# anassinator/pddp

Hardware: AMD Instinct MI355X
Metric: pddp_iterations_per_sec (higher is better)
Workload: dtype f32; 1 GPU; BASELINE.json configs[1]: cartpole n=4 m=1, known-dynamics iLQR, horizon=100, batch=4096 trajectories per GPU, bounds +-10 (eig-clamp + BoxQP branch), 10 line-search alphas; batch_per_gpu=4096, horizon=100, alphas=10, launch_form=10 rounds per launch, rounds_per_launch=10, backward_kernel_variant=0

## Files before the change

pddp_amd/csrc/accept.hpp:

```cpp
#pragma once

#include "pddp_common.hpp"

namespace pddp {

template <typename T>
struct AcceptArgs {
  int B, N, n, m, A;
  const T* Zc;
  const T* Uc;
  const T* Jc;
  const T* gains;
  const int32_t* bwd_status;
  double tol, max_reg;
  int n_iterations;
  T* Z;
  T* U;
  T* gains_acc;
  T* J_opt;
  double* mu;
  double* delta;
  int32_t* state;
  int32_t* iter;
  uint8_t* active;
  uint8_t* fresh;
  int32_t* n_live;
};

constexpr double kMuMin = 1e-6;
constexpr double kDelta0 = 2.0;

constexpr int kAcceptThreads = 64;
constexpr int kMaxAlphas = 16;
constexpr int kLiveShards = 256;


template <typename T>
struct AcceptIn {
  int bstat, iter;
  double mu, delta;
  T J_opt;
};
template <typename T>
PDDP_DEV AcceptIn<T> accept_load(const AcceptArgs<T>& a, int b) {
  AcceptIn<T> in;
  in.bstat = a.bwd_status[b];
  in.mu = a.mu[b];
  in.delta = a.delta[b];
  in.J_opt = a.J_opt[b];
  in.iter = a.iter[b];
  return in;
}

template <typename T>
PDDP_DEV int argmin_first(const T* J, int A, T& Jm_out) {
  int amin = 0;
  T Jm = J[0];
#pragma unroll
  for (int i = 1; i < kMaxAlphas; ++i) {
    const bool take = (i < A) && (Jm == Jm) && (J[i] < Jm || J[i] != J[i]);
    amin = take ? i : amin;
    Jm = take ? J[i] : Jm;
  }
  Jm_out = Jm;
  return amin;
}

template <typename T>
PDDP_DEV int accept_decide(const AcceptArgs<T>& a, int b, const AcceptIn<T>& in,
                           int amin, T J_new, bool& fresh_out) {
  int amin_out = -1;
  double mu = in.mu, delta = in.delta;
  int st;
  bool increase = false;
  if (in.bstat != 0) {
    increase = true;
    st = PDDP_STATE_NOT_PD;
  } else {
    const T J_opt = in.J_opt;
    if (J_new < J_opt) {
      amin_out = amin;
      delta = (delta < 1.0 ? delta : 1.0) / kDelta0;
      mu *= delta;
      if (mu <= kMuMin) mu = 0.0;
      const T rel = abs_(J_opt - J_new) / J_opt;
      st = (rel < (T)a.tol) ? PDDP_STATE_CONVERGED : PDDP_STATE_ACCEPTED;
      a.J_opt[b] = J_new;
    } else {
      increase = true;
      st = PDDP_STATE_REJECTED;
    }
  }
  if (increase) {
    delta = (delta > 1.0 ? delta : 1.0) * kDelta0;
    mu = (kMuMin > mu * delta) ? kMuMin : mu * delta;
    if (mu >= a.max_reg) st = PDDP_STATE_MAX_REG;
  }
  a.mu[b] = mu;
  a.delta[b] = delta;
  a.state[b] = st;
  uint8_t act = 0, fr = 0;
  if (st == PDDP_STATE_NOT_PD || st == PDDP_STATE_REJECTED) {
    act = 1;
  } else if (st == PDDP_STATE_ACCEPTED) {
    if (in.iter < a.n_iterations) {
      a.iter[b] = in.iter + 1;
      act = 1;
      fr = 1;
    }
  }
  a.active[b] = act;
  a.fresh[b] = fr;
  if (act && a.n_live != nullptr)
    atomicAdd(a.n_live + (b & (kLiveShards - 1)), 1);
  fresh_out = fr != 0;
  return amin_out;
}

}
```

pddp_amd/csrc/line_search_lds.hpp:

```cpp
#pragma once

#include <type_traits>
#include "models.hpp"
#include "problem_args.hpp"
#include "accept.hpp"
#include "riccati_n4.hpp"

namespace pddp {

template <typename T>
PDDP_DEV void group_copy(T* dst, const T* src, int count, int l16) {
  constexpr int kDeep = 8;
  for (int o0 = l16; o0 < count; o0 += 16 * kDeep) {
    T tmp[kDeep];
#pragma unroll
    for (int r = 0; r < kDeep; ++r) {
      const int o = o0 + 16 * r;
      tmp[r] = src[o < count ? o : 0];
    }
#pragma unroll
    for (int r = 0; r < kDeep; ++r) {
      const int o = o0 + 16 * r;
      if (o < count) dst[o] = tmp[r];
    }
  }
}

PDDP_DEV void store4(float* p, float a, float b, float c, float d) {
  *reinterpret_cast<float4*>(p) = make_float4(a, b, c, d);
}
PDDP_DEV void store4(double* p, double a, double b, double c, double d) {
  *reinterpret_cast<double2*>(p) = make_double2(a, b);
  *reinterpret_cast<double2*>(p + 2) = make_double2(c, d);
}

template <typename T, int n, int m>
PDDP_DEV void control_law(const T* z, const T* zr, const T* gr, const T* us,
                          T alpha, const T* umin, const T* umax, T* un) {
#pragma unroll
  for (int r = 0; r < m; ++r) {
    T s = T(0);
#pragma unroll
    for (int c = 0; c < n; ++c)
      s = n4::fma_(z[c] - zr[c], gr[m + r * n + c], s);
    const T du = n4::fma_(alpha, gr[r], s);
    const T v = us[r] + du;
    un[r] = clamp_nan(v, umin[r], umax[r]);
  }
}

#ifdef PDDP_WG_TIMELINE
__device__ long long g_search_timeline[1024][12];
#define PDDP_TLS(I)                                                           \
  do {                                                                        \
    if ((threadIdx.x & 255) == 0 && blockIdx.x < 1024)                        \
      g_search_timeline[blockIdx.x][(I) + 4 * (threadIdx.x >> 8)] =           \
          wall_clock64();                                                     \
  } while (0)
#define PDDP_TLS_AT(SLOT)                                                     \
  do {                                                                        \
    if (threadIdx.x == 0 && blockIdx.x < 1024)                                \
      g_search_timeline[blockIdx.x][SLOT] = wall_clock64();                   \
  } while (0)
#else
#define PDDP_TLS(I)
#define PDDP_TLS_AT(SLOT)
#endif

template <typename T>
struct PreStaged {
  const T* Zs;
  const T* Us;
  const T* Gs;
  int status;
  T J_opt;
  T* carry_rows = nullptr;
};
template <typename T, int MODEL, bool FUSED, int WPB, int H, unsigned QM,
          bool DENSE, bool PRE = false>
PDDP_DEV void line_search_lds_body(const ProblemT<T> P,
                                   const LineSearchArgs<T> a,
                                   const AcceptArgs<T> c, T* rec, T* Lout,
                                   unsigned char* smem_raw,
                                   const PreStaged<T> pre,
                                   const unsigned tid = threadIdx.x) {
  using D = ModelDims<MODEL>;
  constexpr int n = D::n, m = D::m;
  constexpr int GS = m + m * n;
  static_assert(H == 1 || (H == 2 && FUSED), "");
  static_assert(!DENSE || (FUSED && H == 1), "");
  static_assert(!PRE || (FUSED && H == 2 && !DENSE), "");
  constexpr int GST = PRE ? GS + m : GS;
  constexpr int UST = PRE ? GS + m : m;
  constexpr int kTailRows = DENSE ? 8 : 4;
  __shared__ int sh_dec[WPB][4][2];
  const int lane = tid & (kWave - 1);
  const int wave_all = tid >> 6;
  const int wave = H == 1 ? wave_all : wave_all % WPB;
  const int hid = H == 1 ? 0 : wave_all / WPB;
  const int grp = lane >> 4, ai = lane & 15;
  const int N = a.N;
  const int per = DENSE ? N * GS : (N + 1) * n + N * m + N * GS;
  T* smem = reinterpret_cast<T*>(smem_raw) + (size_t)wave * 4 * per;
  const int b0 = (blockIdx.x * WPB + wave) * 4;
  PDDP_TLS(0);

  for (int g = 0; g < (PRE ? 0 : 4); ++g) {
    const int bg = b0 + g;
    if (bg >= a.B) break;
    if (H == 2 && (g & 1) != hid) continue;
    if (a.active != nullptr && a.active[bg] == 0) continue;
    T* dst = smem + (size_t)g * per;
    const T* zs = a.Z + (size_t)bg * (N + 1) * n;
    const T* us = a.U + (size_t)bg * N * m;
    const T* gs = a.gains + (size_t)bg * N * GS;
    if constexpr (DENSE) {
      for (int o = lane; o < N * GS; o += kWave) dst[o] = gs[o];
    } else {
      for (int o = lane; o < (N + 1) * n; o += kWave) dst[o] = zs[o];
      for (int o = lane; o < N * m; o += kWave) dst[(N + 1) * n + o] = us[o];
      for (int o = lane; o < N * GS; o += kWave)
        dst[(N + 1) * n + N * m + o] = gs[o];
    }
  }
  if constexpr (!PRE) __syncthreads();
  PDDP_TLS(1);

  const int b = b0 + grp;
  const bool exists = b < a.B;
  const int bc = exists ? b : a.B - 1;
  const bool attempted =
      exists && (a.active == nullptr || a.active[bc] != 0);
  const bool run =
      attempted && ai < a.A &&
      (PRE ? pre.status == 0
           : (a.bwd_status == nullptr || a.bwd_status[bc] == 0));
  if constexpr (!FUSED) {
    if (!run) return;
  }
  const bool bounded = a.u_min != nullptr && a.u_max != nullptr;
  T umin[m], umax[m];
#pragma unroll
  for (int r = 0; r < m; ++r) {
    umin[r] = bounded ? a.u_min[r] : -(T)__builtin_inff();
    umax[r] = bounded ? a.u_max[r] : (T)__builtin_inff();
  }
  const T* Zs = PRE ? pre.Zs
                    : DENSE ? a.Z + (size_t)bc * (N + 1) * n
                            : smem + (size_t)grp * per;
  const T* Us = PRE ? pre.Us
                    : DENSE ? a.U + (size_t)bc * N * m : Zs + (N + 1) * n;
  const T* Gs = PRE ? pre.Gs : DENSE ? smem + (size_t)grp * per : Us + N * m;
  const size_t zstep_c = (size_t)a.A * n, ustep_c = (size_t)a.A * m;
  AcceptIn<T> acc_in = {};
  if constexpr (FUSED) {
    if (attempted && ai == 0) {
      acc_in = accept_load(c, b);
      if constexpr (PRE) {
        acc_in.bstat = pre.status;
        acc_in.J_opt = pre.J_opt;
      }
    }
  }
  T Jmine = T(0);
  const bool nocand = FUSED && n <= 4 && Lout == nullptr && rec != nullptr &&
                      a.drop_candidates != 0 && N + 1 <= 16 * H * kTailRows;
  const bool store_uc = !(FUSED && n <= 6 && Lout == nullptr &&
                          rec != nullptr && N + 1 <= 16 * H * kTailRows);
  auto rollout = [&](T alpha, T* Zci, size_t zstep, T* Uci, size_t ustep) {
    T z[n], zn[n], un[m];
#pragma unroll
    for (int j = 0; j < n; ++j) z[j] = Zs[j];
    T J = T(0);
    auto step = [&](const int t) {
      T zr[n], gr[GS], us[m];
      if constexpr (PRE && n == 4) {
        typedef T V4_ __attribute__((ext_vector_type(4)));
        const V4_ v = *reinterpret_cast<const V4_*>(
            __builtin_assume_aligned(Zs + t * 4, 16));
        zr[0] = v[0]; zr[1] = v[1]; zr[2] = v[2]; zr[3] = v[3];
      } else {
#pragma unroll
        for (int j = 0; j < n; ++j) zr[j] = Zs[t * n + j];
      }
      if constexpr (PRE && GST == 6) {
        typedef T V2_ __attribute__((ext_vector_type(2)));
        const V2_* g2 = reinterpret_cast<const V2_*>(
            __builtin_assume_aligned(Gs + t * 6, 8));
        const V2_ a0 = g2[0], a1 = g2[1], a2 = g2[2];
        gr[0] = a0[0]; gr[1] = a0[1]; gr[2] = a1[0]; gr[3] = a1[1];
        gr[4] = a2[0]; us[0] = a2[1];
      } else {
#pragma unroll
        for (int j = 0; j < GS; ++j) gr[j] = Gs[t * GST + j];
#pragma unroll
        for (int j = 0; j < m; ++j) us[j] = Us[t * UST + j];
      }
      const Trig<T, MODEL> tr = trig_of<T, MODEL>(z);
      __builtin_amdgcn_sched_barrier(0);
      if constexpr (PRE) __builtin_amdgcn_s_waitcnt(0xC07F);
      control_law<T, n, m>(z, zr, gr, us, alpha, umin, umax, un);
#pragma unroll
      for (int j = 0; j < n; ++j) Zci[(size_t)t * zstep + j] = z[j];
      if constexpr (!PRE) {
        if (store_uc) {
#pragma unroll
          for (int j = 0; j < m; ++j) Uci[(size_t)t * ustep + j] = un[j];
        }
      }
      J += cost_value<T, MODEL, QM>(P, z, un, tr, false);
      dynamics<T, MODEL, false>(P, z, un, tr, zn, nullptr, nullptr);
#pragma unroll
      for (int j = 0; j < n; ++j) z[j] = zn[j];
    };
    int t = 0;
    if constexpr (n <= 4) {
      for (; t + 3 < N; t += 4) {
        step(t);
        step(t + 1);
        step(t + 2);
        step(t + 3);
      }
    }
#pragma unroll 1
    for (; t < N; ++t) step(t);
#pragma unroll
    for (int j = 0; j < n; ++j) Zci[(size_t)N * zstep + j] = z[j];
    const T lf =
        cost_value<T, MODEL>(P, z, nullptr, trig_of<T, MODEL>(z), true);
    return J + lf;
  };
  if (run && hid == 0) {
    const T alpha = a.alphas[ai];
    const int idx = b * a.A + ai;
    const bool compact0 = FUSED && Lout == nullptr && rec != nullptr &&
                          ai == 0 && n <= 6 && N + 1 <= 16 * H * kTailRows;
    T* Zci = compact0 ? rec + (size_t)b * (N + 1) * n
                      : a.Zc + ((size_t)b * (N + 1) * a.A + ai) * n;
    T* Uci = a.Uc + ((size_t)b * N * a.A + ai) * m;
    const size_t zstep = compact0 ? (size_t)n : (nocand ? 0 : zstep_c);
    const size_t ustep = nocand ? 0 : ustep_c;
    Jmine = rollout(alpha, Zci, zstep, Uci, ustep);
    a.Jc[idx] = Jmine;
  }
  PDDP_TLS(2);

  if constexpr (FUSED) {
    constexpr int kNone = 99;
    const T kInf = (T)__builtin_inff();
    const int nan_first =
        n4::group_min((run && Jmine != Jmine) ? ai : kNone);
    T Jf = (run && Jmine == Jmine) ? Jmine : kInf;
    {
      T y = n4::dpp<0x128>(Jf); Jf = y < Jf ? y : Jf;
      y = n4::dpp<0x12C>(Jf); Jf = y < Jf ? y : Jf;
      y = n4::dpp<(2 | (3 << 2) | (0 << 4) | (1 << 6))>(Jf); Jf = y < Jf ? y : Jf;
      y = n4::dpp<(1 | (0 << 2) | (3 << 4) | (2 << 6))>(Jf); Jf = y < Jf ? y : Jf;
    }
    const int min_first = n4::group_min((run && Jmine == Jf) ? ai : kNone);
    const int amin =
        nan_first != kNone ? nan_first : (min_first != kNone ? min_first : 0);
    const T J_new = nan_first != kNone ? (T)__builtin_nanf("") : Jf;

    int amin_out = -1, fresh_i = 0;
    if (attempted && ai == 0 && hid == 0) {
      bool fr;
      amin_out = accept_decide(c, b, acc_in, amin, J_new, fr);
      fresh_i = fr ? 1 : 0;
    }
    amin_out = __shfl(amin_out, lane & 48);
    fresh_i = __shfl(fresh_i, lane & 48);
    PDDP_TLS_AT(8);
    if constexpr (n <= 4) {
      if (nocand && hid == 0 && __any(amin_out > 0)) {
        if (amin_out > 0 && ai == amin_out)
          rollout(a.alphas[ai], rec + (size_t)b * (N + 1) * n, (size_t)n,
                  a.Uc + ((size_t)b * N * a.A + ai) * m, 0);
      }
    }
    if constexpr (H == 1) {
      if (!__any(amin_out >= 0)) return;
      __builtin_amdgcn_fence(__ATOMIC_ACQ_REL, "workgroup");
    } else {
      if (hid == 0 && ai == 0) {
        sh_dec[wave][grp][0] = amin_out;
        sh_dec[wave][grp][1] = fresh_i;
      }
      __builtin_amdgcn_fence(__ATOMIC_ACQ_REL, "workgroup");
      __syncthreads();
      amin_out = sh_dec[wave][grp][0];
      fresh_i = sh_dec[wave][grp][1];
    }
    PDDP_TLS_AT(9);
    if (amin_out >= 0) {
      constexpr RecLayout lay(n, m);
      constexpr int S = lay.stride;
      const T* srcz = a.Zc + ((size_t)b * (N + 1) * a.A + amin_out) * n;
      const T* srcu = a.Uc + ((size_t)b * N * a.A + amin_out) * m;
      T* Zb = c.Z + (size_t)b * (N + 1) * n;
      T* Ub = c.U + (size_t)b * N * m;
      T* rec_b = rec + (size_t)b * (N + 1) * S;
      T* Ls = PRE ? nullptr : smem + (size_t)grp * per;
      const T* G = c.gains + (size_t)b * N * GS;
      T* Ga = c.gains_acc + (size_t)b * N * GS;
      T zc[n], uc[m];
      const int t_first = ai + 16 * hid;
      constexpr int KR = kTailRows;
      if (n <= 6 && Lout == nullptr && N + 1 <= 16 * H * KR) {
        T zz[KR][n], uu[KR][m];
        const bool from_rec = rec != nullptr && (amin_out == 0 || nocand);
        const T* cz = from_rec ? rec + (size_t)b * (N + 1) * n : srcz;
        const size_t czs = from_rec ? (size_t)n : zstep_c;
#pragma unroll
        for (int k = 0; k < KR; ++k) {
          const int t = t_first + 16 * H * k;
          const int tz = t <= N ? t : N;
#pragma unroll
          for (int j = 0; j < n; ++j) zz[k][j] = cz[(size_t)tz * czs + j];
        }
        const T* Gl = Gs;
        if constexpr (PRE) {
          for (int t = ai + 16 * hid; t < N; t += 16 * H) {
#pragma unroll
            for (int j = 0; j < GS; ++j) Ga[t * GS + j] = Gl[t * GST + j];
          }
        } else {
          constexpr int kDeep = 8;
          int o = ai + 16 * hid;
          for (; o + 16 * H * (kDeep - 1) < N * GS; o += 16 * H * kDeep) {
            T tmp[kDeep];
#pragma unroll
            for (int r = 0; r < kDeep; ++r) tmp[r] = Gl[o + 16 * H * r];
#pragma unroll
            for (int r = 0; r < kDeep; ++r) Ga[o + 16 * H * r] = tmp[r];
          }
          for (; o < N * GS; o += 16 * H) Ga[o] = Gl[o];
        }
        PDDP_TLS_AT(10);
        const T alpha_w = a.alphas[amin_out];
#pragma unroll
        for (int k = 0; k < KR; ++k) {
          const int t = t_first + 16 * H * k;
          const int tu = t < N ? t : 0;
          T zr[n], gr[GS], us[m];
#pragma unroll
          for (int j = 0; j < n; ++j) zr[j] = Zs[tu * n + j];
#pragma unroll
          for (int j = 0; j < GS; ++j) gr[j] = Gs[tu * GST + j];
#pragma unroll
          for (int j = 0; j < m; ++j) us[j] = Us[tu * UST + j];
          control_law<T, n, m>(zz[k], zr, gr, us, alpha_w, umin, umax, uu[k]);
        }
#pragma unroll
        for (int k = 0; k < KR; ++k) {
          const int t = t_first + 16 * H * k;
          if (t <= N) {
#pragma unroll
            for (int j = 0; j < n; ++j) Zb[t * n + j] = zz[k][j];
          }
          if (t < N) {
#pragma unroll
            for (int j = 0; j < m; ++j) Ub[t * m + j] = uu[k][j];
          }
          if constexpr (PRE) {
            if (pre.carry_rows != nullptr && t <= N && N - t <= 16) {
              T* cr = pre.carry_rows + (N - t) * (n + m);
#pragma unroll
              for (int j = 0; j < n; ++j) cr[j] = zz[k][j];
              if (t < N) {
#pragma unroll
                for (int j = 0; j < m; ++j) cr[n + j] = uu[k][j];
              }
            }
          }
        }
      } else {
      {
        const int tz = t_first <= N ? t_first : N;
        const int tu = t_first < N ? t_first : 0;
#pragma unroll
        for (int j = 0; j < n; ++j) zc[j] = srcz[(size_t)tz * zstep_c + j];
#pragma unroll
        for (int j = 0; j < m; ++j) uc[j] = srcu[(size_t)tu * ustep_c + j];
      }
#pragma unroll 1
      for (int t = t_first; t <= N; t += 16 * H) {
        T zn_[n], un_[m];
        {
          const int t2 = t + 16 * H;
          const int tz = t2 <= N ? t2 : N, tu = t2 < N ? t2 : 0;
#pragma unroll
          for (int j = 0; j < n; ++j) zn_[j] = srcz[(size_t)tz * zstep_c + j];
#pragma unroll
          for (int j = 0; j < m; ++j) un_[j] = srcu[(size_t)tu * ustep_c + j];
        }
        const bool terminal = (t == N);
        T un[m];
#pragma unroll
        for (int j = 0; j < m; ++j) un[j] = terminal ? T(0) : uc[j];
#pragma unroll
        for (int j = 0; j < n; ++j) Zb[t * n + j] = zc[j];
        if (!terminal) {
#pragma unroll
          for (int j = 0; j < m; ++j) Ub[t * m + j] = un[j];
        }
        if (fresh_i && Lout != nullptr) {
          T w[S];
          const T l = record_of<T, MODEL>(P, zc, un, terminal, bounded, a.u_min,
                                         a.u_max, w);
          T* dst = rec_b + (size_t)t * S;
#pragma unroll
          for (int j = 0; j < S; j += 4)
            store4(dst + j, w[j], w[j + 1], w[j + 2], w[j + 3]);
          Lout[(size_t)b * (N + 1) + t] = l;
          Ls[t] = l;
        }
#pragma unroll
        for (int j = 0; j < n; ++j) zc[j] = zn_[j];
#pragma unroll
        for (int j = 0; j < m; ++j) uc[j] = un_[j];
      }
      if constexpr (H == 1) {
        group_copy(Ga, G, N * GS, ai);
      } else {
        const int half = (N * GS + 1) / 2;
        const int off = hid * half;
        const int cnt = hid == 0 ? half : N * GS - half;
        group_copy(Ga + off, G + off, cnt, ai);
      }
      }
      if constexpr (H == 1) {
        if (fresh_i && Lout != nullptr) {
          __builtin_amdgcn_fence(__ATOMIC_RELEASE, "wavefront");
          __builtin_amdgcn_wave_barrier();
          if (ai == 0) {
            T Jacc = T(0);
            for (int t = 0; t <= N; ++t) Jacc += Ls[t];
            c.J_opt[b] = Jacc;
            c.fresh[b] = 0;
          }
        }
      }
    }
    if constexpr (H == 2) {
      __syncthreads();
      if (!PRE && amin_out >= 0 && fresh_i && Lout != nullptr && hid == 0 &&
          ai == 0) {
        const T* Ls = smem + (size_t)grp * per;
        T Jacc = T(0);
        for (int t = 0; t <= N; ++t) Jacc += Ls[t];
        c.J_opt[b] = Jacc;
        c.fresh[b] = 0;
      }
    }
  }
  PDDP_TLS(3);
}


template <typename T, int MODEL, bool FUSED, int WPB, int H = 1,
          unsigned QM = kFullMask<MODEL>, bool DENSE = false>
__global__ __launch_bounds__(kWave * WPB * H) __attribute__((
    amdgpu_waves_per_eu((WPB * H >= 8 || DENSE) && sizeof(T) == 4 &&
                                ModelDims<MODEL>::n <= 4
                            ? 4
                            : 1))) void
line_search_lds_kernel(
    ProblemT<T> P, LineSearchArgs<T> a, AcceptArgs<T> c, T* rec, T* Lout) {
  extern __shared__ __attribute__((aligned(16))) unsigned char smem_raw[];
  line_search_lds_body<T, MODEL, FUSED, WPB, H, QM, DENSE>(
      P, a, c, rec, Lout, smem_raw, PreStaged<T>{});
}

}
```

pddp_amd/csrc/riccati_n4_elem.hpp:

```cpp
#pragma once

#include <type_traits>
#include "models.hpp"
#include "riccati_n4_quad.hpp"

namespace pddp {

namespace n4d {
typedef float f32x4 __attribute__((ext_vector_type(4)));
PDDP_DEV int sgn(float x) { return __float_as_int(x); }
PDDP_DEV int splat(int w) {
  int r;
  asm("v_ashrrev_i32 %0, 31, %1" : "=v"(r) : "v"(w));
  return r;
}
PDDP_DEV float bsel(int mask, float a, float b) {
  float r;
  asm("v_bfi_b32 %0, %1, %2, %3" : "=v"(r) : "v"(mask), "v"(a), "v"(b));
  return r;
}

template <typename T>
struct GenArgs {
  const T* Z;
  const T* U;
  T* L;
  T* J_opt;
  uint8_t* fresh;
};
}

namespace n4e {

using n4::bperm;
using n4::dpp;
using n4::fma_;
using n4::group_sum;
using n4::kGain;
using n4::mul_nc;
using n4d::bsel;
using n4d::f32x4;
typedef float f32x2 __attribute__((ext_vector_type(2)));
typedef float f32x3 __attribute__((ext_vector_type(3)));
using n4d::GenArgs;
using n4d::sgn;
using n4d::splat;

constexpr int kWaves = 4;
constexpr int kTrajW = 4;
constexpr int kBlk = 16;
constexpr int kImg = 52;
constexpr int kRowStride = kBlk * kImg + 16;
constexpr int kImgBuf = kTrajW * kRowStride;
constexpr int kTermRow = 24;
constexpr int kTermSh = kTrajW * kTermRow;
constexpr int kPairLdsInl = kImgBuf;
constexpr int kPairLdsOvl = 2 * kImgBuf + kTermSh;

struct LsTableF {
  float v[n4::kLsSteps];
  constexpr LsTableF() : v() {
    for (int n = 0; n < n4::kLsSteps; ++n) v[n] = (float)n4::kLs.v[n];
  }
};
__device__ constexpr LsTableF kLsF{};
template <typename T>
PDDP_DEV const T* ls_table();
template <>
PDDP_DEV const float* ls_table<float>() { return kLsF.v; }
template <>
PDDP_DEV const double* ls_table<double>() { return n4::kLs.v; }
template <typename T>
struct Vec {
  typedef T v4 __attribute__((ext_vector_type(4)));
  typedef T v2 __attribute__((ext_vector_type(2)));
};

struct QpLean1 {
  float x, inv;
  int free_w;
  PDDP_DEV void solve(float x0, float Q, float c, float lo, float hi) {
    const float d_lo = lo - x0, d_hi = x0 - hi;
    const float xs = __builtin_amdgcn_fmed3f(x0, lo, hi);
    const float hQ = 0.5f * Q;
    inv = __builtin_amdgcn_rcpf(Q);
// ... 127 lines not shown
    T kx = qc.x;
    bool Kzero = !qc.free_, fail = qc.fail;
    const bool slow = qc.slow & take;
    if (__any(slow)) {
      unsigned long long todo = __ballot(slow && l == 0);
      while (todo != 0) {
        const int src = __builtin_ctzll(todo);
        todo &= todo - 1;
        const n4::SlowQpOut<T> o = n4q::boxqp1_wave<T, true>(
            __shfl(kprev, src), __shfl(qp_Q, src), __shfl(Qu, src),
            __shfl(lo_b, src), __shfl(hi_b, src), ls_table<T>(), lane);
        const bool mine = (lane >> 4) == (src >> 4);
        kx = mine ? o.x : kx;
        Kzero = mine ? ((o.result_free & 1) == 0) : Kzero;
        fail = mine ? (o.result_free < 2) : fail;
      }
    }
    const T sx = Kzero ? T(0) : qc.inv;
    const int stt = st != PDDP_BWD_OK ? st : (fail ? (int)PDDP_BWD_BOXQP_FAILED : (int)PDDP_BWD_OK);
    T cx, wx;
    n4q::rank_one_coeffs(kx, sx, Quu, Qu, cx, wx);
    kt = take ? kx : kt; sK = take ? sx : sK;
    c = take ? cx : c; wv = take ? wx : wv;
    const bool bad = take & (stt != PDDP_BWD_OK);
    status = bad ? stt : status;
    alive_m &= ~__ballot(bad);
  }
  return ElemGains<T>{kt, sK, c, wv};
}

#ifdef PDDP_ELEM_MARKS
__device__ long long g_elem_marks[8];
#define PDDP_EM_MARK(I) do { if (blockIdx.x == 0 && threadIdx.x == 0) g_elem_marks[I] = clock64(); } while (0)
#define PDDP_EM_ACC(I, T0) do { if (blockIdx.x == 0 && threadIdx.x == 0) g_elem_marks[I] += clock64() - (T0); } while (0)
#define PDDP_EM_NOW() clock64()
#else
#define PDDP_EM_MARK(I)
#define PDDP_EM_ACC(I, T0)
#define PDDP_EM_NOW() 0
#endif

#ifdef PDDP_WG_TIMELINE
__device__ long long g_elem_timeline[1024][12];
#define PDDP_TL(I)                                                            \
  do {                                                                        \
    if ((threadIdx.x & 255) == 0 && blockIdx.x < 1024)                        \
      g_elem_timeline[blockIdx.x][(I) + 4 * (threadIdx.x >> 8)] =             \
          wall_clock64();                                                     \
  } while (0)
#define PDDP_TL_HW(I)                                                         \
  do {                                                                        \
    if (threadIdx.x == 0 && blockIdx.x < 1024) {                              \
      g_elem_timeline[blockIdx.x][8] =                                        \
          __builtin_amdgcn_s_getreg(4 | (0 << 6) | (31 << 11));               \
      g_elem_timeline[blockIdx.x][9] =                                        \
          __builtin_amdgcn_s_getreg(20 | (0 << 6) | (3 << 11));               \
      g_elem_timeline[blockIdx.x][I] = clock64();                             \
    }                                                                         \
  } while (0)
#else
#define PDDP_TL(I)
#define PDDP_TL_HW(I)
#endif

struct RoundOut {
  const float* Zs;
  const float* Gs;
  const float* Us;
  int status;
  float J_opt;
  float* carry_rows;
};
constexpr int round_zu_stride(int N) { return 4 * (N + 1); }
constexpr int kCarryRows = kBlk + 1, kCarryW = 5;
constexpr int kCarryF = kTrajW * kCarryRows * kCarryW;
constexpr int kGainL = kGain + 1;
constexpr int round_gains_floats(int N) { return (kTrajW * N * kGainL + 3) & ~3; }

template <typename T, unsigned QM, bool OVL, bool ROUND>
PDDP_DEV bool elem_sweep_body(const RiccatiArgs<T>& a, const GenArgs<T>& gen,
                              const ProblemT<T>& prob, unsigned char* smem_raw,
                              RoundOut& ro,
                              const unsigned tid = threadIdx.x,
                              const int carry = -1) {
  static_assert(OVL || !ROUND, "");
  constexpr bool F32 = std::is_same<T, float>::value;
  static_assert(F32 || (!OVL && !ROUND), "");
  using V4 = typename Vec<T>::v4;
  using V2 = typename Vec<T>::v2;
  constexpr int MODEL = PDDP_MODEL_CARTPOLE;
  constexpr RecLayout lay(4, 1);
  const int kPairLds = OVL ? kPairLdsOvl + (ROUND ? round_gains_floats(a.N) +
                                                        (carry >= 0 ? kCarryF : 0)
                                                  : 0)
                           : kPairLdsInl;
  const int lane = tid & (kWave - 1);
  const int wave = __builtin_amdgcn_readfirstlane((int)tid >> 6);
  const int pair = OVL ? (wave & (kWaves - 1)) : wave;
  const bool is_gen = OVL && wave >= kWaves;
  T* const img0 = reinterpret_cast<T*>(smem_raw) + pair * kPairLds;
  T* const term_w = OVL ? img0 + 2 * kImgBuf : img0;

  const int row = lane >> 4, l = lane & 15, i = l >> 2, j = l & 3;
  const int N = a.N;
  const int b0 = (blockIdx.x * kWaves + pair) * kTrajW;
  const int b = b0 + row;
  const bool exists = b < a.B;
  const int bc = exists ? b : a.B - 1;
  const T* Zg = gen.Z + (size_t)bc * (size_t)(N + 1) * 4;
  const T* Ug = gen.U + (size_t)bc * (size_t)N;
  const int nblk = (N + kBlk - 1) / kBlk;
  if (b0 >= a.B) return false;
  const bool counted = exists && (a.active == nullptr || a.active[bc] != 0);
  if (!__any(counted)) return false;
  PDDP_EM_MARK(0);
  PDDP_TL(0);
  PDDP_TL_HW(10);
  const T umin = a.u_min[0], umax = a.u_max[0];
  const int rbase = row * kRowStride;

  T zq[4], uq, Jacc = T(0), l_term = T(0);
  [[maybe_unused]] T* const carry_w =
      img0 + kPairLdsOvl + (ROUND ? round_gains_floats(N) : 0) +
      row * kCarryRows * kCarryW;
  if constexpr (ROUND) ro.carry_rows = carry >= 0 ? carry_w : nullptr;
  auto request = [&](int jb) {
    int tau = N - 1 - kBlk * jb - l;
    tau = tau < 0 ? 0 : tau;
    if constexpr (ROUND) {
      if (jb == 0 && carry == 0) {
        const T* cr = carry_w + (N - tau) * kCarryW;
        zq[0] = cr[0]; zq[1] = cr[1]; zq[2] = cr[2]; zq[3] = cr[3];
        uq = cr[4];
        return;
      }
    }
    const V4 v = *reinterpret_cast<const V4*>(Zg + 4 * tau);
    zq[0] = v[0]; zq[1] = v[1]; zq[2] = v[2]; zq[3] = v[3];
    uq = Ug[tau];
    if constexpr (ROUND) {
      if (jb == 0 && carry == 1 && N - tau <= kBlk) {
        T* cr = carry_w + (N - tau) * kCarryW;
        cr[0] = zq[0]; cr[1] = zq[1]; cr[2] = zq[2]; cr[3] = zq[3];
        cr[4] = uq;
      }
    }
  };
  auto terminal = [&]() {
    T zN[4];
    if (ROUND && carry == 0) {
      zN[0] = carry_w[0]; zN[1] = carry_w[1]; zN[2] = carry_w[2];
      zN[3] = carry_w[3];
    } else {
      const V4 zNv = *reinterpret_cast<const V4*>(Zg + 4 * N);
      zN[0] = zNv[0]; zN[1] = zNv[1]; zN[2] = zNv[2]; zN[3] = zNv[3];
      if (ROUND && carry == 1 && l == 0) {
        carry_w[0] = zN[0]; carry_w[1] = zN[1]; carry_w[2] = zN[2];
        carry_w[3] = zN[3];
      }
    }
    T lz[4], lzz[16], lu[1], luu[1];
    l_term = cost_derivs<T, MODEL>(prob, zN, nullptr, trig_of<T, MODEL>(zN),
                                   true, lz, lzz, lu, luu);
    T* scr = term_w + row * kTermRow;
    if (l == 0) {
#pragma unroll
      for (int k = 0; k < 16; k += 4)
        *reinterpret_cast<V4*>(scr + k) =
            V4{lzz[k], lzz[k + 1], lzz[k + 2], lzz[k + 3]};
      *reinterpret_cast<V4*>(scr + 16) = V4{lz[0], lz[1], lz[2], lz[3]};
      scr[20] = l_term;
      if (counted) gen.L[(size_t)bc * (size_t)(N + 1) + N] = l_term;
    }
  };
  auto pass = [&](int jb, T* buf) {
    const T z[4] = {zq[0], zq[1], zq[2], zq[3]};
    const T u = uq;
    if (jb + 1 < nblk) request(jb + 1);
    const int tau = N - 1 - kBlk * jb - l;
    T w[lay.stride];
    const T lc = record_of<T, MODEL, QM>(prob, z, &u, false, true, a.u_min,
                                         a.u_max, w);
    T* dst = buf + rbase + l * kImg;
#pragma unroll
    for (int r = 0; r < 4; ++r)
      *reinterpret_cast<V4*>(dst + 4 * r) =
          V4{w[lay.oFz + ((r + 0) & 3) * 4 + r],
                w[lay.oFz + ((r + 1) & 3) * 4 + r],
                w[lay.oFz + ((r + 2) & 3) * 4 + r],
                w[lay.oFz + ((r + 3) & 3) * 4 + r]};
#pragma unroll
    for (int x = 0; x < 4; x += 2) {
      *reinterpret_cast<V4*>(dst + 16 + 2 * x) =
          V4{w[lay.oFu + x], w[lay.oLuz + x], w[lay.oFu + x + 1],
                w[lay.oLuz + x + 1]};
      *reinterpret_cast<V4*>(dst + 24 + 2 * x) =
          V4{w[lay.oFu + x], w[lay.oLz + x], w[lay.oFu + x + 1],
                w[lay.oLz + x + 1]};
    }
#pragma unroll
    for (int r = 0; r < 4; ++r)
      *reinterpret_cast<V4*>(dst + 32 + 4 * r) =
          V4{w[lay.oLzz + 4 * r], w[lay.oLzz + 4 * r + 1],
                w[lay.oLzz + 4 * r + 2], w[lay.oLzz + 4 * r + 3]};
    *reinterpret_cast<V4*>(dst + 48) =
        V4{w[lay.oLuu], w[lay.oLu], umin - w[lay.oU], umax - w[lay.oU]};
    if (tau >= 0) {
      if (counted) gen.L[(size_t)bc * (size_t)(N + 1) + tau] = lc;
      Jacc += lc;
    }
  };
  auto finish_costs = [&]() {
    const bool sums = counted && (gen.fresh == nullptr || gen.fresh[bc] != 0);
    const T Jrow = group_sum(Jacc) + (OVL ? term_w[row * kTermRow + 20] : l_term);
    if constexpr (ROUND) {
      const T Jold = gen.J_opt[bc];
      if (l == 0) term_w[row * kTermRow + 21] = sums ? Jrow : Jold;
    }
    if (sums && l == 0) {
      gen.J_opt[bc] = Jrow;
      if (gen.fresh != nullptr) gen.fresh[bc] = 0;
    }
  };
  [[maybe_unused]] T* const gains_w = img0 + kPairLdsOvl;
  auto flush_gains = [&](const T* ib, int t_top, int cnt) {
    const T* sg = ib + l * kImg + rbase;
    const V4 Kv = *reinterpret_cast<const V4*>(sg);
    const T kv = sg[4];
    if (exists && l < cnt) {
      T* g = a.gains + ((size_t)bc * (size_t)N + (size_t)(t_top - l)) * kGain;
      g[0] = kv; g[1] = Kv[0]; g[2] = Kv[1]; g[3] = Kv[2]; g[4] = Kv[3];
      if constexpr (ROUND) {
        T* gl = gains_w + (row * N + (t_top - l)) * kGainL;
        gl[0] = kv; gl[1] = Kv[0]; gl[2] = Kv[1]; gl[3] = Kv[2]; gl[4] = Kv[3];
      }
    }
  };
  [[maybe_unused]] T* const zu_w =
      img0 + (nblk & 1) * kImgBuf + row * round_zu_stride(N);
  [[maybe_unused]] auto round_out = [&](int status_) {
    if constexpr (ROUND) {
      ro.Zs = zu_w;
      ro.Gs = gains_w + row * N * kGainL;
      ro.Us = ro.Gs + kGain;
      ro.status = status_;
      n4::lds_publish_barrier();
      ro.J_opt = term_w[row * kTermRow + 21];
    }
  };
  if constexpr (OVL) {
    if (is_gen) {
      request(0);
      pass(0, img0);
      PDDP_TL(1);
      n4::lds_publish_barrier();
      for (int jb = 1; jb < nblk; ++jb) {
        if (jb >= 2)
          flush_gains(img0 + (jb & 1) * kImgBuf, N - 1 - kBlk * (jb - 2), kBlk);
        pass(jb, img0 + (jb & 1) * kImgBuf);
        n4::lds_publish_barrier();
      }
      if (nblk >= 2)
        flush_gains(img0 + (nblk & 1) * kImgBuf, N - 1 - kBlk * (nblk - 2), kBlk);
      if constexpr (ROUND) {
        asm volatile("s_waitcnt lgkmcnt(0)" ::: "memory");
        constexpr int kCh = 8;
        V4 zc[kCh];
        T uc[kCh];
#pragma unroll
        for (int c = 0; c < kCh; ++c) {
          const int tz = l + 16 * c;
          zc[c] = *reinterpret_cast<const V4*>(Zg + 4 * (tz <= N ? tz : N));
          uc[c] = Ug[tz < N ? tz : 0];
        }
#pragma unroll
        for (int c = 0; c < kCh; ++c) {
          const int tz = l + 16 * c;
          if (tz <= N) *reinterpret_cast<V4*>(zu_w + 4 * tz) = zc[c];
          if (tz < N) gains_w[(row * N + tz) * kGainL + kGain] = uc[c];
        }
      }
      finish_costs();
      PDDP_TL(3);
      if constexpr (ROUND) round_out(PDDP_BWD_OK);
      return true;
    }
  }

  const T reg = (T)a.reg[bc];
  const int oA = rbase + 4 * i, oB = rbase + 4 * j, oL = rbase + 32 + l;
  const int oTi = rbase + 16 + 2 * i, oTj = rbase + 24 + 2 * j;
  const int tr_addr = ((lane & 48) | (j * 4 + i)) * 4;
  if constexpr (OVL) {
    __builtin_amdgcn_s_setprio(3);
    terminal();
    n4::lds_publish_barrier();
  } else {
    request(0);
    terminal();
    asm volatile("s_waitcnt lgkmcnt(0)" ::: "memory");
  }
  T V = term_w[row * kTermRow + l];
  T vc = term_w[row * kTermRow + 16 + j];

  struct Words {
    V4 Fs, Fq;
    V2 Ti, Tj;
    V4 Sc;
    T Lzz;
  };
  auto gather = [&](const T* ib, const int s) {
    const T* p = ib + s * kImg;
    Words w;
    w.Fs = *reinterpret_cast<const V4*>(p + oA);
    w.Fq = *reinterpret_cast<const V4*>(p + oB);
    w.Ti = *reinterpret_cast<const V2*>(p + oTi);
    w.Tj = *reinterpret_cast<const V2*>(p + oTj);
    w.Lzz = p[oL];
    w.Sc = *reinterpret_cast<const V4*>(p + 48 + rbase);
    return w;
  };
  T kprev = T(0);
  int status = PDDP_BWD_OK;
  unsigned long long alive_m = __ballot(counted);
  const int ostage = rbase + l;

  auto step = [&](const Words& w, T* ib, const int s) {
    const StepCoreT<T> q = step_core(V, vc, w.Ti[0], w.Tj[0], w.Fs, w.Fq,
                                     w.Lzz, w.Tj[1], w.Ti[1], w.Sc[0], w.Sc[1]);
    const T Quu = q.Quu, Qu = q.Qu;
    const T QzzT = bperm(tr_addr, q.Qzz);
    const T Quzc = bperm(tr_addr, q.Quzr);
    __builtin_amdgcn_sched_barrier(0);
    const ElemGains<T> g_ = elem_gains<T>(kprev, Quu, Qu, reg, w.Sc[2], w.Sc[3],
                                          lane, status, alive_m);
    const T kt = g_.kt, sK = g_.sK, c = g_.c, wv = g_.wv;
    ib[s * kImg + ostage] = (l < 4) ? -(sK * Quzc) : kt;
    kprev = kt;
    V = fma_(T(0.5), n4::opaque(q.Qzz + QzzT),
             mul_nc(c, mul_nc(q.Quzr, Quzc)));
    vc = fma_(wv, Quzc, q.Qzc);
  };

  PDDP_EM_MARK(1);
  PDDP_TL(1);
  int t = N - 1;
  for (int jb = 0; jb < nblk; ++jb) {
    T* ib = img0;
    if constexpr (OVL) {
      ib = img0 + (jb & 1) * kImgBuf;
    } else {
      [[maybe_unused]] const long long tp0 = PDDP_EM_NOW();
      pass(jb, img0);
      asm volatile("s_waitcnt lgkmcnt(0)" ::: "memory");
      PDDP_EM_ACC(4, tp0);
    }
    [[maybe_unused]] const long long ts0 = PDDP_EM_NOW();
    Words wa = gather(ib, 0), wb = wa;
    if (t >= kBlk - 1) {
#pragma unroll
      for (int s = 0; s < kBlk; s += 2) {
        wb = gather(ib, s + 1);
        step(wa, ib, s);
        if (s + 2 < kBlk) wa = gather(ib, s + 2);
        step(wb, ib, s + 1);
      }
      asm volatile("s_waitcnt lgkmcnt(0)" ::: "memory");
      if (!OVL || jb + 1 == nblk) flush_gains(ib, t, kBlk);
      t -= kBlk;
    } else {
      const int cnt = t + 1;
#pragma unroll 1
      for (int s = 0; s < cnt; ++s) {
        const Words w = gather(ib, s);
        step(w, ib, s);
      }
      asm volatile("s_waitcnt lgkmcnt(0)" ::: "memory");
      flush_gains(ib, t, cnt);
      t = -1;
    }
    asm volatile("s_waitcnt lgkmcnt(0)" ::: "memory");
    PDDP_EM_ACC(5, ts0);
    if constexpr (OVL) {
      if (jb + 1 < nblk) {
        [[maybe_unused]] const long long tb0 = PDDP_EM_NOW();
        n4::lds_publish_barrier();
        PDDP_EM_ACC(6, tb0);
      }
    }
  }
  PDDP_EM_MARK(2);
  PDDP_TL(2);
  if (counted && l == 0) a.status[bc] = status;
  if constexpr (!OVL) finish_costs();
  PDDP_EM_MARK(3);
  PDDP_TL(3);
  PDDP_TL_HW(11);
  if constexpr (ROUND) round_out(status);
  return true;
}

template <unsigned QM, bool OVL>
__global__ __launch_bounds__((OVL ? 2 : 1) * kWaves * kWave) void
riccati_n4_elem_kernel(RiccatiArgs<float> a, GenArgs<float> gen,
                       ProblemT<float> prob) {
  extern __shared__ __attribute__((aligned(16))) unsigned char smem_raw[];
  RoundOut ro;
  elem_sweep_body<float, QM, OVL, false>(a, gen, prob, smem_raw, ro);
}
template <unsigned QM>
__global__ __launch_bounds__(kWaves * kWave) void riccati_n4_elem_f64_kernel(
    RiccatiArgs<double> a, GenArgs<double> gen, ProblemT<double> prob) {
  extern __shared__ __attribute__((aligned(16))) unsigned char smem_raw[];
  RoundOut ro;
  elem_sweep_body<double, QM, false, false>(a, gen, prob, smem_raw, ro);
}

}

inline int& nominal_kernel_choice() {
  static int choice = 0;
  return choice;
}

static int launch_n4_elem(const pddp_problem& p, const RiccatiArgs<float>& a,
                          const n4d::GenArgs<float>& gen, hipStream_t st,
                          int overlap = -1) {
  if (p.model != PDDP_MODEL_CARTPOLE ||
      p.encoding != PDDP_ENC_IGNORE_UNCERTAINTY || a.u_min == nullptr ||
      a.u_max == nullptr || a.branch != PDDP_BRANCH_EIG || a.N < 1)
    return PDDP_E_UNSUPPORTED;
  const ProblemT<float> P = convert_problem<float>(p);
  constexpr int kPer = n4e::kWaves * n4e::kTrajW;
  const dim3 grid((a.B + kPer - 1) / kPer);
  const bool ovl = overlap < 0 ? grid.x <= 256u : overlap != 0;
  constexpr unsigned kSparse = 0b11001u;
  const bool sparse =
      (live_mask(p.Q, ModelDims<PDDP_MODEL_CARTPOLE>::na) & ~kSparse) == 0;
#define PDDP_ELEM_GO(QMV, OV)                                                 \
  do {                                                                        \
    auto kern = n4e::riccati_n4_elem_kernel<QMV, OV>;                         \
    const size_t lds = (size_t)n4e::kWaves * sizeof(float) *                  \
                       (OV ? n4e::kPairLdsOvl : n4e::kPairLdsInl);            \
    const hipError_t e = hipFuncSetAttribute(                                 \
        (const void*)kern, hipFuncAttributeMaxDynamicSharedMemorySize,        \
        (int)lds);                                                            \
    if (e != hipSuccess) return (int)e;                                       \
    PDDP_LAUNCH(kern, grid, dim3((OV ? 2 : 1) * n4e::kWaves * kWave), lds,    \
                st, a, gen, P);                                               \
  } while (0)
  constexpr unsigned kFull = kFullMask<PDDP_MODEL_CARTPOLE>;
  if (sparse) { if (ovl) PDDP_ELEM_GO(kSparse, true); else PDDP_ELEM_GO(kSparse, false); }
  else { if (ovl) PDDP_ELEM_GO(kFull, true); else PDDP_ELEM_GO(kFull, false); }
#undef PDDP_ELEM_GO
  return launch_status();
}

static int launch_n4_elem_f64(const pddp_problem& p,
                              const RiccatiArgs<double>& a,
                              const n4d::GenArgs<double>& gen, hipStream_t st) {
  if (p.model != PDDP_MODEL_CARTPOLE ||
      p.encoding != PDDP_ENC_IGNORE_UNCERTAINTY || a.u_min == nullptr ||
      a.u_max == nullptr || a.branch != PDDP_BRANCH_EIG || a.N < 1)
    return PDDP_E_UNSUPPORTED;
  const ProblemT<double> P = convert_problem<double>(p);
  constexpr int kPer = n4e::kWaves * n4e::kTrajW;
  const dim3 grid((a.B + kPer - 1) / kPer);
  constexpr unsigned kSparse = 0b11001u;
  constexpr unsigned kFull = kFullMask<PDDP_MODEL_CARTPOLE>;
// ... 20 lines not shown
```

pddp_amd/csrc/round_n4.hip:

```cpp
#include "riccati_n4_elem.hpp"
#include "line_search_lds.hpp"

namespace pddp {

template <unsigned QM, bool MULTI>
__global__ __launch_bounds__(2 * n4e::kWaves * kWave) void round_n4_kernel(
    RiccatiArgs<float> a, n4d::GenArgs<float> gen, ProblemT<float> prob,
    LineSearchArgs<float> ls, AcceptArgs<float> ac, float* scratch,
    int rounds, long long* phase_ticks, int use_carry) {
  extern __shared__ __attribute__((aligned(16))) unsigned char smem_raw[];
  const bool timed = phase_ticks != nullptr && threadIdx.x == 0;
  long long t_sweep = 0, t_search = 0;
  for (int r = 0;; ++r) {
    int z = 0;
    unsigned tid = threadIdx.x;
    if constexpr (MULTI) {
      asm volatile("s_mov_b32 %0, 0" : "=s"(z));
      asm volatile("" : "+v"(tid));
    }
    RiccatiArgs<float> a_r = a;
    a_r.N += z;
    LineSearchArgs<float> ls_r = ls;
    ls_r.N += z;
    AcceptArgs<float> ac_r = ac;
    ac_r.N += z;
    n4e::RoundOut ro;
    const long long t0 = timed ? wall_clock64() : 0;
    const int carry = MULTI && use_carry ? (r == 0 ? 1 : 0) : -1;
    if (!n4e::elem_sweep_body<float, QM, true, true>(a_r, gen, prob, smem_raw,
                                                     ro, tid, carry))
      break;
    const long long t1 = timed ? wall_clock64() : 0;
    const PreStaged<float> pre{ro.Zs, ro.Us,      ro.Gs,
                               ro.status, ro.J_opt, ro.carry_rows};
    line_search_lds_body<float, PDDP_MODEL_CARTPOLE, true, n4e::kWaves, 2, QM,
                         false, true>(prob, ls_r, ac_r, scratch, nullptr,
                                      smem_raw, pre, tid);
    if (timed) {
      t_sweep += t1 - t0;
      t_search += wall_clock64() - t1;
    }
    if (!MULTI || r + 1 >= rounds) break;
    __builtin_amdgcn_fence(__ATOMIC_ACQ_REL, "workgroup");
    __syncthreads();
  }
  if (timed) {
    phase_ticks[2 * blockIdx.x] += t_sweep;
    phase_ticks[2 * blockIdx.x + 1] += t_search;
  }
}

static int launch_round_n4(const pddp_problem& p, const RiccatiArgs<float>& a,
                           const n4d::GenArgs<float>& gen,
                           const LineSearchArgs<float>& ls,
                           const AcceptArgs<float>& ac, float* scratch,
                           int rounds, long long* phase_ticks,
                           hipStream_t st) {
  if (p.model != PDDP_MODEL_CARTPOLE ||
      p.encoding != PDDP_ENC_IGNORE_UNCERTAINTY || a.u_min == nullptr ||
      a.u_max == nullptr || a.branch != PDDP_BRANCH_EIG || a.N < 1 ||
      a.N + 1 > 128 || ls.A > 16 || rounds < 1)
    return PDDP_E_UNSUPPORTED;
  constexpr int kPer = n4e::kWaves * n4e::kTrajW;
  const dim3 grid((a.B + kPer - 1) / kPer);
  if (grid.x > 256u) return PDDP_E_UNSUPPORTED;
  const size_t lds0 = (size_t)n4e::kWaves * sizeof(float) *
                      (n4e::kPairLdsOvl + n4e::round_gains_floats(a.N));
  const size_t lds1 = lds0 + (size_t)n4e::kWaves * sizeof(float) * n4e::kCarryF;
  const int use_carry = rounds > 1 && lds1 <= 159 * 1024;
  const size_t lds = use_carry ? lds1 : lds0;
  if (lds > 159 * 1024) return PDDP_E_UNSUPPORTED;
  const ProblemT<float> P = convert_problem<float>(p);
  constexpr unsigned kSparse = 0b11001u;
  constexpr unsigned kFull = kFullMask<PDDP_MODEL_CARTPOLE>;
  const bool sparse =
      (live_mask(p.Q, ModelDims<PDDP_MODEL_CARTPOLE>::na) & ~kSparse) == 0;
#define PDDP_ROUND_GO(QMV)                                                    \
  do {                                                                        \
    auto kern = rounds > 1 ? round_n4_kernel<QMV, true>                       \
                           : round_n4_kernel<QMV, false>;                     \
    const hipError_t e = hipFuncSetAttribute(                                 \
        (const void*)kern, hipFuncAttributeMaxDynamicSharedMemorySize,        \
        (int)lds);                                                            \
    if (e != hipSuccess) return (int)e;                                       \
    PDDP_LAUNCH(kern, grid, dim3(2 * n4e::kWaves * kWave), lds, st, a, gen,   \
                P, ls, ac, scratch, rounds, phase_ticks, use_carry);          \
  } while (0)
  if (sparse) PDDP_ROUND_GO(kSparse); else PDDP_ROUND_GO(kFull);
#undef PDDP_ROUND_GO
  return launch_status();
}

}

extern "C" int pddp_round_nominal_f32(
    const pddp_problem* problem, int B, int N, int A, float* Z, float* U,
    const float* alphas, const float* u_min, const float* u_max, int branch,
    uint8_t* active, uint8_t* fresh, float* gains, int32_t* bwd_status,
    float* L, float* J_opt, float* Zc, float* Uc, float* Jc, double tol,
    double max_reg, int n_iterations, float* gains_acc, double* mu,
    double* delta, int32_t* state, int32_t* iter, int32_t* n_live,
    float* scratch, int rounds, long long* phase_ticks, void* stream) {
  if (problem == nullptr || B <= 0 || N <= 0 || A <= 0 || !Z || !U || !alphas ||
      !active || !fresh || !gains || !bwd_status || !L || !J_opt || !Zc ||
      !Uc || !Jc || !gains_acc || !mu || !delta || !state || !iter || !scratch)
    return PDDP_E_BADARG;
  if (branch != PDDP_BRANCH_EIG && branch != PDDP_BRANCH_CHOLESKY)
    return PDDP_E_BADARG;
  pddp::RiccatiArgs<float> a;
  a.B = B; a.N = N; a.n = 4;
  a.rec = nullptr;
  a.u_min = u_min; a.u_max = u_max;
  a.reg = mu;
  a.branch = branch;
  a.active = active;
  a.gains = gains;
  a.status = bwd_status;
  const pddp::n4d::GenArgs<float> gen = {Z, U, L, J_opt, fresh};
  const pddp::LineSearchArgs<float> ls{B, N, A, Z, U, gains, alphas, u_min,
                                       u_max, active, bwd_status, Zc, Uc, Jc};
  const pddp::AcceptArgs<float> ac{
      B, N, 4, 1, A, Zc, Uc, Jc, gains, bwd_status, tol, max_reg, n_iterations,
      Z, U, gains_acc, J_opt, mu, delta, state, iter, active, fresh, n_live};
  return pddp::launch_round_n4(*problem, a, gen, ls, ac, scratch, rounds,
                               phase_ticks, (hipStream_t)stream);
}

// ... 11 lines not shown
```

Measured before the change: 46.28 million trajectory-iterations/s.

## Carry per-trajectory accept state and next-round rows in LDS across rounds

Adds a RoundCarry struct (mu, delta, J_opt, flags) that the fused line-search/accept writes to shared memory. The next round's Riccati sweep and line search read active/fresh/mu/J_opt/iter from it instead of global memory. The chosen rollout's z/u rows are also written directly into the gains LDS region, so the next sweep reads them locally rather than from global Z/U. The end-of-round full workgroup fence plus syncthreads becomes a lighter LDS publish barrier, with one full sync kept inside the sweep. The goal is to cut global loads and barriers between rounds, at the cost of more intricate cross-phase LDS ownership that could race if the barriers are insufficient.

```diff
diff --git a/pddp_amd/csrc/accept.hpp b/pddp_amd/csrc/accept.hpp
--- a/pddp_amd/csrc/accept.hpp
+++ b/pddp_amd/csrc/accept.hpp
@@ -53,6 +53,13 @@
 }
 
 template <typename T>
+struct RoundCarry {
+  double mu, delta;
+  T J_opt;
+  int flags;
+};
+
+template <typename T>
 PDDP_DEV int argmin_first(const T* J, int A, T& Jm_out) {
   int amin = 0;
   T Jm = J[0];
@@ -68,7 +75,8 @@
 
 template <typename T>
 PDDP_DEV int accept_decide(const AcceptArgs<T>& a, int b, const AcceptIn<T>& in,
-                           int amin, T J_new, bool& fresh_out) {
+                           int amin, T J_new, bool& fresh_out,
+                           RoundCarry<T>* carry = nullptr) {
   int amin_out = -1;
   double mu = in.mu, delta = in.delta;
   int st;
@@ -100,11 +108,13 @@
   a.delta[b] = delta;
   a.state[b] = st;
   uint8_t act = 0, fr = 0;
+  int iter = in.iter;
   if (st == PDDP_STATE_NOT_PD || st == PDDP_STATE_REJECTED) {
     act = 1;
   } else if (st == PDDP_STATE_ACCEPTED) {
     if (in.iter < a.n_iterations) {
-      a.iter[b] = in.iter + 1;
+      iter = in.iter + 1;
+      a.iter[b] = iter;
       act = 1;
       fr = 1;
     }
@@ -114,6 +124,9 @@
   if (act && a.n_live != nullptr)
     atomicAdd(a.n_live + (b & (kLiveShards - 1)), 1);
   fresh_out = fr != 0;
+  if (carry != nullptr)
+    *carry = RoundCarry<T>{mu, delta, amin_out >= 0 ? J_new : in.J_opt,
+                           act | (fr << 1) | (iter << 2)};
   return amin_out;
 }
 
diff --git a/pddp_amd/csrc/line_search_lds.hpp b/pddp_amd/csrc/line_search_lds.hpp
--- a/pddp_amd/csrc/line_search_lds.hpp
+++ b/pddp_amd/csrc/line_search_lds.hpp
@@ -75,6 +75,9 @@
   int status;
   T J_opt;
   T* carry_rows = nullptr;
+  const RoundCarry<T>* carry_in = nullptr;
+  RoundCarry<T>* carry_out = nullptr;
+  T* next_rows = nullptr;
 };
 template <typename T, int MODEL, bool FUSED, int WPB, int H, unsigned QM,
           bool DENSE, bool PRE = false>
@@ -130,7 +133,9 @@
   const bool exists = b < a.B;
   const int bc = exists ? b : a.B - 1;
   const bool attempted =
-      exists && (a.active == nullptr || a.active[bc] != 0);
+      exists && (PRE && pre.carry_in != nullptr
+                     ? (pre.carry_in[grp].flags & 1) != 0
+                     : (a.active == nullptr || a.active[bc] != 0));
   const bool run =
       attempted && ai < a.A &&
       (PRE ? pre.status == 0
@@ -153,14 +158,23 @@
   const T* Gs = PRE ? pre.Gs : DENSE ? smem + (size_t)grp * per : Us + N * m;
   const size_t zstep_c = (size_t)a.A * n, ustep_c = (size_t)a.A * m;
   AcceptIn<T> acc_in = {};
-  if constexpr (FUSED) {
-    if (attempted && ai == 0) {
-      acc_in = accept_load(c, b);
-      if constexpr (PRE) {
-        acc_in.bstat = pre.status;
-        acc_in.J_opt = pre.J_opt;
-      }
-    }
+  if constexpr (PRE) {
+    if (exists && ai == 0 && hid == 0) {
+      if (pre.carry_in != nullptr) {
+        const RoundCarry<T> k = pre.carry_in[grp];
+        acc_in.mu = k.mu;
+        acc_in.delta = k.delta;
+        acc_in.iter = k.flags >> 2;
+      } else if (attempted || pre.carry_out != nullptr) {
+        acc_in.mu = c.mu[b];
+        acc_in.delta = c.delta[b];
+        acc_in.iter = c.iter[b];
+      }
+      acc_in.bstat = pre.status;
+      acc_in.J_opt = pre.J_opt;
+    }
+  } else if constexpr (FUSED) {
+    if (attempted && ai == 0) acc_in = accept_load(c, b);
   }
   T Jmine = T(0);
   const bool nocand = FUSED && n <= 4 && Lout == nullptr && rec != nullptr &&
@@ -265,8 +279,15 @@
     int amin_out = -1, fresh_i = 0;
     if (attempted && ai == 0 && hid == 0) {
       bool fr;
-      amin_out = accept_decide(c, b, acc_in, amin, J_new, fr);
+      RoundCarry<T> next;
+      amin_out = accept_decide(c, b, acc_in, amin, J_new, fr, &next);
       fresh_i = fr ? 1 : 0;
+      if constexpr (PRE) {
+        if (pre.carry_out != nullptr) pre.carry_out[grp] = next;
+      }
+    } else if (PRE && pre.carry_out != nullptr && ai == 0 && hid == 0) {
+      pre.carry_out[grp] = RoundCarry<T>{acc_in.mu, acc_in.delta, acc_in.J_opt,
+                                         acc_in.iter << 2};
     }
     amin_out = __shfl(amin_out, lane & 48);
     fresh_i = __shfl(fresh_i, lane & 48);
@@ -372,6 +393,13 @@
                 for (int j = 0; j < m; ++j) cr[n + j] = uu[k][j];
               }
             }
+            if (pre.next_rows != nullptr && t < N) {
+              T* nr = pre.next_rows + t * GST;
+#pragma unroll
+              for (int j = 0; j < n; ++j) nr[j] = zz[k][j];
+#pragma unroll
+              for (int j = 0; j < m; ++j) nr[GS + j] = uu[k][j];
+            }
           }
         }
       } else {
@@ -438,6 +466,18 @@
             for (int t = 0; t <= N; ++t) Jacc += Ls[t];
             c.J_opt[b] = Jacc;
             c.fresh[b] = 0;
+          }
+        }
+      }
+    }
+    if constexpr (PRE) {
+      if (pre.next_rows != nullptr && amin_out < 0) {
+#pragma unroll
+        for (int k = 0; k < kTailRows; ++k) {
+          const int t = ai + 16 * hid + 16 * H * k;
+          if (t < N) {
+#pragma unroll
+            for (int j = 0; j < n; ++j) pre.next_rows[t * GST + j] = Zs[t * n + j];
           }
         }
       }
diff --git a/pddp_amd/csrc/riccati_n4_elem.hpp b/pddp_amd/csrc/riccati_n4_elem.hpp
--- a/pddp_amd/csrc/riccati_n4_elem.hpp
+++ b/pddp_amd/csrc/riccati_n4_elem.hpp
@@ -1,6 +1,7 @@
 #pragma once
 
 #include <type_traits>
+#include "accept.hpp"
 #include "models.hpp"
 #include "riccati_n4_quad.hpp"
 
@@ -294,7 +295,8 @@
                               const ProblemT<T>& prob, unsigned char* smem_raw,
                               RoundOut& ro,
                               const unsigned tid = threadIdx.x,
-                              const int carry = -1) {
+                              const int carry = -1,
+                              const RoundCarry<T>* rc = nullptr) {
   static_assert(OVL || !ROUND, "");
   constexpr bool F32 = std::is_same<T, float>::value;
   static_assert(F32 || (!OVL && !ROUND), "");
@@ -323,7 +325,11 @@
   const T* Ug = gen.U + (size_t)bc * (size_t)N;
   const int nblk = (N + kBlk - 1) / kBlk;
   if (b0 >= a.B) return false;
-  const bool counted = exists && (a.active == nullptr || a.active[bc] != 0);
+  const bool later = ROUND && carry == 0;
+  const RoundCarry<T>* const rcm = later ? rc + pair * kTrajW + row : nullptr;
+  const bool counted =
+      exists && (later ? (rcm->flags & 1) != 0
+                       : (a.active == nullptr || a.active[bc] != 0));
   if (!__any(counted)) return false;
   PDDP_EM_MARK(0);
   PDDP_TL(0);
@@ -336,6 +342,7 @@
       img0 + kPairLdsOvl + (ROUND ? round_gains_floats(N) : 0) +
       row * kCarryRows * kCarryW;
   if constexpr (ROUND) ro.carry_rows = carry >= 0 ? carry_w : nullptr;
+  [[maybe_unused]] T* const gains_w = img0 + kPairLdsOvl;
   auto request = [&](int jb) {
     int tau = N - 1 - kBlk * jb - l;
     tau = tau < 0 ? 0 : tau;
@@ -344,6 +351,14 @@
         const T* cr = carry_w + (N - tau) * kCarryW;
         zq[0] = cr[0]; zq[1] = cr[1]; zq[2] = cr[2]; zq[3] = cr[3];
         uq = cr[4];
+        return;
+      }
+      if (carry == 0) {
+        const V2* g2 = reinterpret_cast<const V2*>(
+            gains_w + (row * N + tau) * kGainL);
+        const V2 z01 = g2[0], z23 = g2[1];
+        zq[0] = z01[0]; zq[1] = z01[1]; zq[2] = z23[0]; zq[3] = z23[1];
+        uq = gains_w[(row * N + tau) * kGainL + kGain];
         return;
       }
     }
@@ -423,10 +438,12 @@
     }
   };
   auto finish_costs = [&]() {
-    const bool sums = counted && (gen.fresh == nullptr || gen.fresh[bc] != 0);
+    const bool sums =
+        counted && (later ? (rcm->flags & 2) != 0
+                          : (gen.fresh == nullptr || gen.fresh[bc] != 0));
     const T Jrow = group_sum(Jacc) + (OVL ? term_w[row * kTermRow + 20] : l_term);
     if constexpr (ROUND) {
-      const T Jold = gen.J_opt[bc];
+      const T Jold = later ? rcm->J_opt : gen.J_opt[bc];
       if (l == 0) term_w[row * kTermRow + 21] = sums ? Jrow : Jold;
     }
     if (sums && l == 0) {
@@ -434,7 +451,6 @@
       if (gen.fresh != nullptr) gen.fresh[bc] = 0;
     }
   };
-  [[maybe_unused]] T* const gains_w = img0 + kPairLdsOvl;
   auto flush_gains = [&](const T* ib, int t_top, int cnt) {
     const T* sg = ib + l * kImg + rbase;
     const V4 Kv = *reinterpret_cast<const V4*>(sg);
@@ -460,17 +476,24 @@
       ro.J_opt = term_w[row * kTermRow + 21];
     }
   };
+  const int sync_at = nblk >= 2 ? 1 : 0;
+  [[maybe_unused]] auto block_barrier = [&](int k) {
+    if (later && k == sync_at)
+      __syncthreads();
+    else
+      n4::lds_publish_barrier();
+  };
   if constexpr (OVL) {
     if (is_gen) {
       request(0);
       pass(0, img0);
       PDDP_TL(1);
-      n4::lds_publish_barrier();
+      block_barrier(0);
       for (int jb = 1; jb < nblk; ++jb) {
         if (jb >= 2)
           flush_gains(img0 + (jb & 1) * kImgBuf, N - 1 - kBlk * (jb - 2), kBlk);
         pass(jb, img0 + (jb & 1) * kImgBuf);
-        n4::lds_publish_barrier();
+        block_barrier(jb);
       }
       if (nblk >= 2)
         flush_gains(img0 + (nblk & 1) * kImgBuf, N - 1 - kBlk * (nblk - 2), kBlk);
@@ -483,13 +506,13 @@
         for (int c = 0; c < kCh; ++c) {
           const int tz = l + 16 * c;
           zc[c] = *reinterpret_cast<const V4*>(Zg + 4 * (tz <= N ? tz : N));
-          uc[c] = Ug[tz < N ? tz : 0];
+          uc[c] = later ? T(0) : Ug[tz < N ? tz : 0];
         }
 #pragma unroll
         for (int c = 0; c < kCh; ++c) {
           const int tz = l + 16 * c;
           if (tz <= N) *reinterpret_cast<V4*>(zu_w + 4 * tz) = zc[c];
-          if (tz < N) gains_w[(row * N + tz) * kGainL + kGain] = uc[c];
+          if (!later && tz < N) gains_w[(row * N + tz) * kGainL + kGain] = uc[c];
         }
       }
       finish_costs();
@@ -499,14 +522,14 @@
     }
   }
 
-  const T reg = (T)a.reg[bc];
+  const T reg = later ? (T)rcm->mu : (T)a.reg[bc];
   const int oA = rbase + 4 * i, oB = rbase + 4 * j, oL = rbase + 32 + l;
   const int oTi = rbase + 16 + 2 * i, oTj = rbase + 24 + 2 * j;
   const int tr_addr = ((lane & 48) | (j * 4 + i)) * 4;
   if constexpr (OVL) {
     __builtin_amdgcn_s_setprio(3);
     terminal();
-    n4::lds_publish_barrier();
+    block_barrier(0);
   } else {
     request(0);
     terminal();
@@ -596,7 +619,7 @@
     if constexpr (OVL) {
       if (jb + 1 < nblk) {
         [[maybe_unused]] const long long tb0 = PDDP_EM_NOW();
-        n4::lds_publish_barrier();
+        block_barrier(jb + 1);
         PDDP_EM_ACC(6, tb0);
       }
     }
diff --git a/pddp_amd/csrc/round_n4.hip b/pddp_amd/csrc/round_n4.hip
--- a/pddp_amd/csrc/round_n4.hip
+++ b/pddp_amd/csrc/round_n4.hip
@@ -2,6 +2,7 @@
 #include "line_search_lds.hpp"
 
 namespace pddp {
+
 
 template <unsigned QM, bool MULTI>
 __global__ __launch_bounds__(2 * n4e::kWaves * kWave) void round_n4_kernel(
@@ -9,6 +10,7 @@
     LineSearchArgs<float> ls, AcceptArgs<float> ac, float* scratch,
     int rounds, long long* phase_ticks, int use_carry) {
   extern __shared__ __attribute__((aligned(16))) unsigned char smem_raw[];
+  __shared__ RoundCarry<float> sh_carry[2][n4e::kWaves * n4e::kTrajW];
   const bool timed = phase_ticks != nullptr && threadIdx.x == 0;
   long long t_sweep = 0, t_search = 0;
   for (int r = 0;; ++r) {
@@ -27,12 +29,24 @@
     n4e::RoundOut ro;
     const long long t0 = timed ? wall_clock64() : 0;
     const int carry = MULTI && use_carry ? (r == 0 ? 1 : 0) : -1;
+    RoundCarry<float>* const rc_in = carry == 0 ? sh_carry[r & 1] : nullptr;
+    RoundCarry<float>* const rc_out =
+        carry >= 0 ? sh_carry[(r + 1) & 1] : nullptr;
     if (!n4e::elem_sweep_body<float, QM, true, true>(a_r, gen, prob, smem_raw,
-                                                     ro, tid, carry))
+                                                     ro, tid, carry, rc_in))
       break;
     const long long t1 = timed ? wall_clock64() : 0;
-    const PreStaged<float> pre{ro.Zs, ro.Us,      ro.Gs,
-                               ro.status, ro.J_opt, ro.carry_rows};
+    const int pair = (tid >> 6) & (n4e::kWaves - 1);
+    const PreStaged<float> pre{
+        ro.Zs,
+        ro.Us,
+        ro.Gs,
+        ro.status,
+        ro.J_opt,
+        ro.carry_rows,
+        rc_in ? rc_in + pair * n4e::kTrajW : nullptr,
+        rc_out ? rc_out + pair * n4e::kTrajW : nullptr,
+        carry >= 0 ? const_cast<float*>(ro.Gs) : nullptr};
     line_search_lds_body<float, PDDP_MODEL_CARTPOLE, true, n4e::kWaves, 2, QM,
                          false, true>(prob, ls_r, ac_r, scratch, nullptr,
                                       smem_raw, pre, tid);
@@ -41,8 +55,12 @@
       t_search += wall_clock64() - t1;
     }
     if (!MULTI || r + 1 >= rounds) break;
-    __builtin_amdgcn_fence(__ATOMIC_ACQ_REL, "workgroup");
-    __syncthreads();
+    if (carry >= 0) {
+      n4::lds_publish_barrier();
+    } else {
+      __builtin_amdgcn_fence(__ATOMIC_ACQ_REL, "workgroup");
+      __syncthreads();
+    }
   }
   if (timed) {
     phase_ticks[2 * blockIdx.x] += t_sweep;
```

Result: no change. 46.39 million trajectory-iterations/s, median of 6 (+0.2%).
